# EnricoMiccoli/nodal

Hardware: AMD Instinct MI355X
Metric: circuits_per_sec (higher is better)
Workload: dtype f64; 1 GPU; cfg3: grid(1000) 1e6 nodes, sparse CSR path; n=999999, nnz=4995995, parallelism=one GPU

## Files before the change

nodal_amd/csrc/sagg.hip:

```cpp
#include <hip/hip_ext.h>

#include <atomic>
#include <type_traits>

#include "group.h"

int grounded_flags(nodal_ctx *h, uint8_t *flags_dev);

namespace {

using grp::TB;
constexpr int PW = 4;
constexpr int ACAP = 64;
constexpr int RCAP = 96;
constexpr int RCAP_SMALL = 512;
constexpr int RCAP_SMALL_ROWS = 16384;
inline int rcap_for(int64_t nc) { return nc <= RCAP_SMALL_ROWS ? RCAP_SMALL : RCAP; }
constexpr int W0_MAX = 32;
constexpr int COARSEST = 64;
constexpr int MAX_LEVELS = 12;
constexpr int MIS_ROUNDS = 6;
constexpr int TAIL_MAX_N = 1024;
constexpr int TAIL_LEVELS = 6;
constexpr int TAIL_LDS_BUDGET = 150 * 1024;
// ... 2 lines not shown
#ifndef NODAL_SA_OMEGA
#define NODAL_SA_OMEGA 0.85
#endif
constexpr double OMEGA = NODAL_SA_OMEGA;
constexpr double OMEGA_P = 0.70;
constexpr double OMEGA_P_COARSE = 0.85;
using cyc_t = nodal_cyc_t;

inline unsigned grid_for(int64_t n, unsigned cap = 8192) {
    int64_t g = (n + TB - 1) / TB;
    if (g < 1) g = 1;
    if (g >= 64) g = (g + 7) & ~(int64_t)7;
    return (unsigned)(g > cap ? cap : g);
}
inline int64_t pad64(int64_t n) { return (n + 63) & ~(int64_t)63; }

__device__ __forceinline__ unsigned xcd_block() {
    const unsigned g = gridDim.x, b = blockIdx.x;
    return (g & 7u) ? b : (b & 7u) * (g >> 3) + (b >> 3);
}


struct Ell {
    int64_t n = 0, ld = 0;
    int32_t width = 0;
    const int32_t *col = nullptr;
    const int16_t *dcol = nullptr;
    const double *val = nullptr;
    const float *valf = nullptr;
    const int32_t *len = nullptr;
};

enum { ST_MAXLEN = 0, ST_GRADED = 1, ST_BADDIAG = 2, ST_OVERFLOW = 3, ST_NNZ = 4, ST_UNASSIGNED = 5,
       ST_MAXR = 6, ST_NC = 7 ,
       ST_FARCOL = 8 , ST_COUNT = 9 };

struct SLevel {
    int64_t n = 0, ld = 0, nc = 0;
    int32_t width = 0;
    int32_t maxlen = 0;
    int32_t wfix = 0;
    int64_t nnz = 0;
    DevBuf acol, aval, alen, dinv;
    DevBuf adcol;
    bool d16 = false;
    DevBuf agg, pcol, pval;
    DevBuf rcol, rval, rlen;
    int64_t rld = 0;
    DevBuf vec, part, gflag;
    DevBuf avalf, pvalf, rvalf;
    Ell A() const {
        Ell e;
        e.n = n; e.ld = ld; e.width = width;
        e.col = acol.as<int32_t>(); e.val = aval.as<double>(); e.len = alen.as<int32_t>();
        e.valf = avalf.as<float>();
        e.dcol = d16 ? adcol.as<int16_t>() : nullptr;
        return e;
    }
    template <typename T = double> T *v(int which) const { return reinterpret_cast<T *>(vec.as<double>() + (int64_t)which * ld); }
};
enum { V_X = 0, V_R = 1, V_XP = 2, V_RC = 3, V_C1 = 4, V_C2 = 5, V_V1 = 6, V_V2 = 7, V_R2 = 8, V_X1 = 9, V_T = 10,
       V_COUNT = 11 };

struct TailLevelDesc {
    int n, nc, ld, rld, width, nq, lpr;
// ... 61 lines not shown
        if (it_exec) (void)hipGraphExecDestroy(it_exec);
        if (it_graph) (void)hipGraphDestroy(it_graph);
        it_exec = nullptr;
        it_graph = nullptr;
        it_key = 0;
    }
    ~SHierarchy() {
        drop_graph();
        if (ev_copy) (void)hipEventDestroy(ev_copy);
        if (ev_fork) (void)hipEventDestroy(ev_fork);
        if (ev_join) (void)hipEventDestroy(ev_join);
        if (ev_flags) (void)hipEventDestroy(ev_flags);
        if (aux) (void)hipStreamDestroy(aux);
        for (SLevel *l : pool) {
            DevBuf *b[] = {&l->acol, &l->aval, &l->alen, &l->dinv, &l->agg, &l->pcol, &l->pval, &l->rcol,
                           &l->rval, &l->rlen, &l->vec, &l->part, &l->gflag, &l->avalf, &l->pvalf, &l->rvalf, &l->adcol};
            for (DevBuf *x : b) x->release();
            delete l;
        }
        tail_image.release();
        tail_op.release();
        mvec.release();
        tail_stamps.release();
        bstat.release();
        apcol.release();
        apval.release();
        aplen.release();
        DevBuf *b[] = {&stats, &coarse_inv, &mis_t, &mis_m, &mis_flag, &mis_id, &agg1, &keys, &rstart, &cursor, &lists};
        for (DevBuf *x : b) x->release();
        if (host_stats) (void)hipHostFree(host_stats);
    }
// ... 455 lines not shown
    }
}

__device__ __forceinline__ int wave_excl_scan(int v, int *total) {
    const int lane = threadIdx.x & 63;
    int incl = v;
#pragma unroll
    for (int off = 1; off < 64; off <<= 1) {
        const int t = __shfl_up(incl, off, 64);
        if (lane >= off) incl += t;
    }
    *total = __shfl(incl, 63, 64);
    return incl - v;
}

template <int APW>
__global__ __launch_bounds__(TB) void ap_rows(Ell A, const int32_t *__restrict__ pcol, const double *__restrict__ pval,
                                              int32_t *__restrict__ apcol, double *__restrict__ apval,
                                              int32_t *__restrict__ aplen, unsigned long long *__restrict__ stats) {
    bool overflow = false;
    for (int64_t i = (int64_t)xcd_block() * TB + threadIdx.x; i < A.n; i += (int64_t)gridDim.x * TB) {
        int32_t c[APW];
        double v[APW];
#pragma unroll
        for (int q = 0; q < APW; ++q) { c[q] = -1; v[q] = 0.0; }
        int cnt = 0;
        const int32_t l = A.len[i];
        for (int32_t s = 0; s < l; ++s) {
            const int32_t k = A.col[(int64_t)s * A.ld + i];
            const double a = A.val[(int64_t)s * A.ld + i];
            int32_t J[PW];
            double pp[PW];
#pragma unroll
            for (int sp = 0; sp < PW; ++sp) {
                J[sp] = pcol[(int64_t)sp * A.ld + k];
                pp[sp] = pval[(int64_t)sp * A.ld + k];
            }
#pragma unroll
// ... 5 lines not shown
                for (int q = 0; q < APW; ++q)
                    if (!placed && c[q] == J[sp]) { v[q] += t; placed = true; }
#pragma unroll
                for (int q = 0; q < APW; ++q)
                    if (!placed && c[q] < 0) { c[q] = J[sp]; v[q] = t; placed = true; cnt = q + 1; }
                if (!placed) overflow = true;
            }
        }
#pragma unroll
        for (int q = 0; q < APW; ++q)
            if (q < cnt) {
                apcol[(int64_t)q * A.ld + i] = c[q];
                apval[(int64_t)q * A.ld + i] = v[q];
            }
        aplen[i] = cnt;
    }
    if (overflow) atomicOr(&stats[ST_OVERFLOW], 4ull);
}

template <int APW>
__global__ __launch_bounds__(64) void ap_rows_lds(Ell A, const int32_t *__restrict__ pcol,
                                                  const double *__restrict__ pval, int32_t *__restrict__ apcol,
                                                  double *__restrict__ apval, int32_t *__restrict__ aplen,
                                                  unsigned long long *__restrict__ stats) {
    __shared__ int32_t tc[APW * 64];
    __shared__ double tv[APW * 64];
    const int lane = threadIdx.x;
    bool overflow = false;
    for (int64_t i0 = (int64_t)xcd_block() * 64; i0 < A.n; i0 += (int64_t)gridDim.x * 64) {
        const int64_t i = i0 + lane;
#pragma unroll 8
        for (int q = 0; q < APW; ++q) tc[q * 64 + lane] = -1;
        int cnt = 0;
        if (i < A.n) {
            const int32_t l = A.len[i];
            constexpr int AB = 4;
            for (int32_t s0 = 0; s0 < l; s0 += AB) {
                int32_t kk[AB];
                double aa[AB];
#pragma unroll
                for (int u = 0; u < AB; ++u) {
                    const int32_t su = s0 + u < l ? s0 + u : 0;
                    kk[u] = A.col[(int64_t)su * A.ld + i];
                    aa[u] = A.val[(int64_t)su * A.ld + i];
                }
                int32_t J[AB][PW];
                double pp[AB][PW];
#pragma unroll
                for (int u = 0; u < AB; ++u)
#pragma unroll
// ... 15 lines not shown
                            if (c == J[u][sp]) {
                                tv[slot * 64 + lane] += t;
                                placed = true;
                            } else if (c < 0) {
                                tc[slot * 64 + lane] = J[u][sp];
                                tv[slot * 64 + lane] = t;
                                ++cnt;
                                placed = true;
                            }
                            slot = (slot + 1) & (APW - 1);
                        }
                        if (!placed) overflow = true;
                    }
                }
            }
            int o = 0;
            for (int q = 0; q < APW; ++q) {
                const int32_t c = tc[q * 64 + lane];
                if (c >= 0) {
                    apcol[(int64_t)o * A.ld + i] = c;
                    apval[(int64_t)o * A.ld + i] = tv[q * 64 + lane];
                    ++o;
                }
            }
            aplen[i] = cnt;
        }
    }
    if (overflow) atomicOr(&stats[ST_OVERFLOW], 4ull);
}

__device__ __forceinline__ int galerkin_products(int64_t ld, const int32_t *__restrict__ apcol,
                                                 const double *__restrict__ apval, const int32_t *__restrict__ aplen,
                                                 int64_t rld, const int32_t *__restrict__ rcol,
                                                 const double *__restrict__ rval, int64_t I, int t0, int tn,
                                                 int32_t *lJ, double *lV) {
    const int lane = threadIdx.x;
    int32_t i = 0, len = 0;
    double w = 0.0;
    if (lane < tn) {
        const int t = t0 + lane;
        const int64_t rat = ((int64_t)(t >> 3) * rld + I) * 8 + (t & 7);
        i = rcol[rat];
        w = rval[rat];
// ... 269 lines not shown
    hipStream_t st = h->stream;
    SLevel *L = H->level(l), *C = H->level(l + 1);
    const int64_t n = L->n, ld = L->ld, nc = C->n;
    Ell A = L->A();
    A.width = L->maxlen;
    unsigned long long *dstats = H->stats.as<unsigned long long>();
    const int apw = A.width <= 6 ? 16 : 64;
    NODAL_HIP_TRY(h, H->apcol.reserve((size_t)apw * ld * 4 + 64));
    NODAL_HIP_TRY(h, H->apval.reserve((size_t)apw * ld * 8 + 64));
    NODAL_HIP_TRY(h, H->aplen.reserve((size_t)ld * 4 + 64));
    int32_t *apcol = H->apcol.as<int32_t>(), *aplen = H->aplen.as<int32_t>();
    double *apval = H->apval.as<double>();
    unsigned long long *lst = dstats + (size_t)l * ST_COUNT;
    const unsigned g = grid_for(n);
    if (phase != 2) {
        switch (apw) {
        case 16: ap_rows<16><<<g, TB, 0, st>>>(A, L->pcol.as<int32_t>(), L->pval.as<double>(), apcol, apval, aplen, lst); break;
        default: {
            const unsigned gl = (unsigned)((n + 63) / 64 < 4096 ? (n + 63) / 64 : 4096);
            ap_rows_lds<64><<<gl, 64, 0, st>>>(A, L->pcol.as<int32_t>(), L->pval.as<double>(), apcol, apval, aplen, lst);
        } break;
        }
        NODAL_HIP_TRY(h, hipGetLastError());
    }
    if (phase == 1) return NODAL_OK;
    int G = 1024 / apw;
    G = (G < 8 ? 8 : (G > 64 ? 64 : G));
    static const int g_env = getenv("NODAL_SA_GG") ? atoi(getenv("NODAL_SA_GG")) : 40;
    if (g_env >= 8 && g_env <= 64 && apw == 16) G = g_env & ~7;
    const int pcap = G * apw + 72;
    const size_t lds = 1024 + (size_t)pcap * 12;
    static const int64_t gcap = getenv("NODAL_SA_GCAP") ? atoll(getenv("NODAL_SA_GCAP")) : 16384;
    static const int maxseg = getenv("NODAL_SA_GSEG") ? atoi(getenv("NODAL_SA_GSEG")) : 4;
    const unsigned gg = (unsigned)(nc < gcap ? nc : (gcap < BSTAT_MAX ? gcap : BSTAT_MAX));
    if (r_ready) NODAL_HIP_TRY(h, hipStreamWaitEvent(st, r_ready, 0));
    galerkin<NUMERIC><<<gg, 64, lds, st>>>(
        ld, apcol, apval, aplen, nc, L->rld, L->rcol.as<int32_t>(), L->rval.as<double>(), L->rlen.as<int32_t>(),
// ... 7 lines not shown
}

double omega_p(int level) {
    static double w[2] = {-1.0, -1.0};
    if (w[0] < 0.0) {
        double a = OMEGA_P, b = OMEGA_P_COARSE;
        if (const char *e = getenv("NODAL_SA_OMEGA_P")) {
            a = atof(e);
            const char *c = strchr(e, ',');
            b = c ? atof(c + 1) : a;
        }
        w[1] = b > 0.0 && b < 1.2 ? b : OMEGA_P_COARSE;
        w[0] = a > 0.0 && a < 1.0 ? a : OMEGA_P;
    }
    return w[level > 0 ? 1 : 0];
}

int build_level(nodal_ctx *h, SHierarchy *H, int l, unsigned long long *hs, bool *declined, bool *stop) {
    hipStream_t st = h->stream;
    SLevel *L = H->level(l);
    const int64_t n = L->n, ld = L->ld;
    Ell A = L->A();
    A.width = L->maxlen;
    unsigned long long *dstats = H->stats.as<unsigned long long>();

    NODAL_HIP_TRY(h, H->mis_t.reserve((size_t)n * 8 + 64));
    NODAL_HIP_TRY(h, H->mis_m.reserve((size_t)n * 8 + 64));
    NODAL_HIP_TRY(h, H->mis_flag.reserve((size_t)(n + 1) * 4 + 64));
    NODAL_HIP_TRY(h, H->mis_id.reserve((size_t)(n + 1) * 4 + 64 + scan_tmp_bytes(n + 1)));
    NODAL_HIP_TRY(h, H->agg1.reserve((size_t)n * 4 + 64));
// ... 99 lines not shown
    NODAL_HIP_TRY(h, L->rlen.reserve((size_t)C->ld * 4 + 64));
    NODAL_HIP_TRY(h, C->acol.reserve((size_t)ACAP * C->ld * 4 + 64));
    NODAL_HIP_TRY(h, C->aval.reserve((size_t)ACAP * C->ld * 8 + 64));
    NODAL_HIP_TRY(h, C->avalf.reserve((size_t)ACAP * C->ld * 4 + 64));
    NODAL_HIP_TRY(h, C->alen.reserve((size_t)C->ld * 4 + 64));
    NODAL_HIP_TRY(h, C->dinv.reserve((size_t)C->ld * 8 + 64));
    if (forked && H->want_flags) {
        if (l == 0) NODAL_HIP_TRY(h, L->gflag.reserve((size_t)n + 64));
        NODAL_HIP_TRY(h, C->gflag.reserve((size_t)C->n + 64));
    }
    {
        const int apw = L->maxlen <= 6 ? 16 : 64;
        NODAL_HIP_TRY(h, H->apcol.reserve((size_t)apw * ld * 4 + 64));
        NODAL_HIP_TRY(h, H->apval.reserve((size_t)apw * ld * 8 + 64));
        NODAL_HIP_TRY(h, H->aplen.reserve((size_t)ld * 4 + 64));
    }
    hipStream_t main_st = h->stream;
    struct StreamGuard {
        nodal_ctx *h;
        hipStream_t keep;
        ~StreamGuard() { h->stream = keep; }
    } guard{h, main_st};
    if (forked) {
        NODAL_HIP_TRY(h, hipEventRecord(H->ev_fork, main_st));
        NODAL_HIP_TRY(h, hipStreamWaitEvent(H->aux, H->ev_fork, 0));
        H->aux_pending = true;
        NODAL_TRY(galerkin_product<false>(h, H, l, nullptr, 1));
        h->stream = H->aux;
        st = H->aux;
    }
// ... 125 lines not shown
        NODAL_HIP_TRY(h, hipDeviceGetAttribute(&ncu, hipDeviceAttributeMultiprocessorCount, h->device >= 0 ? h->device : 0));
        if (ncu < 1) ncu = 1;
        cus[dev].store(ncu, std::memory_order_release);
    }
    NODAL_HIP_TRY(h, H->tail_op.reserve((size_t)n * n * 8 + 64));
    const unsigned gr = (unsigned)(n < ncu ? n : ncu);
    double *T = H->tail_op.as<double>();
    const char *img = H->tail_image.as<char>();
    if (d.slots <= 8) k_tail_pack_op<8><<<gr, 1024, (size_t)d.lds_bytes, h->stream>>>(d, img, T);
    else if (d.slots <= 16) k_tail_pack_op<16><<<gr, 1024, (size_t)d.lds_bytes, h->stream>>>(d, img, T);
    else k_tail_pack_op<32><<<gr, 1024, (size_t)d.lds_bytes, h->stream>>>(d, img, T);
    NODAL_HIP_TRY(h, hipGetLastError());
    H->tail_dense = true;
    static const bool check = getenv("NODAL_TRACE") && getenv("NODAL_SA_TAIL_CHECK") && atoi(getenv("NODAL_SA_TAIL_CHECK")) != 0;
    if (check) NODAL_TRY(tail_self_check(h, H));
    return NODAL_OK;
}

int build_tail(nodal_ctx *h, SHierarchy *H, const unsigned long long *hs) {
    H->tail = -1;
    H->tail_dense = false;
    const int last = H->nlev - 1;
    auto up16 = [](int x) { return (x + 15) & ~15; };
    for (int t = 1; t <= last; ++t) {
        if (H->pool[t]->n > TAIL_MAX_N || last - t + 1 > TAIL_LEVELS) continue;
        TailDesc d;
        memset(&d, 0, sizeof d);
        d.nlev = last - t + 1;
        d.nu = getenv("NODAL_SA_TAIL_NU") ? atoi(getenv("NODAL_SA_TAIL_NU")) : 3;
        if (d.nu < 1) d.nu = 1;
// ... 109 lines not shown
        NODAL_TRY(galerkin_product<true>(h, H, l, forked ? H->ev_join : nullptr, forked ? 2 : 0));
        if (forked) H->aux_pending = false;
    }
    const int last = H->nlev - 1;
    if (H->dense_coarsest)
        coarsest_inverse<<<1, 256, 0, st>>>(H->pool[last]->A(), H->coarse_inv.as<double>(), dstats + (size_t)last * ST_COUNT);
    if (H->tail >= 0) k_tail_pack<<<1, 1024, 0, st>>>(H->td, H->tail_image.as<char>());
    NODAL_HIP_TRY(h, hipGetLastError());
    NODAL_TRY(form_tail_op(h, H));
    NODAL_HIP_TRY(h, hipMemcpyAsync(hs, dstats, (size_t)MAX_LEVELS * ST_COUNT * 8, hipMemcpyDeviceToHost, st));
    NODAL_WAIT_STREAM(h, st);
    const int64_t bar = n0 / 100 < 32 ? (n0 / 100 > 0 ? n0 / 100 : 1) : 32;
    if (hs[ST_BADDIAG] || (int64_t)hs[ST_GRADED] >= bar) return NODAL_OK;
    for (int k = 1; k < H->nlev; ++k)
        if (hs[(size_t)k * ST_COUNT + ST_BADDIAG] || hs[(size_t)k * ST_COUNT + ST_OVERFLOW]) return NODAL_OK;
    *ok = true;
    return NODAL_OK;
}

}

void sagg_destroy(nodal_ctx *h) {
    delete static_cast<SHierarchy *>(h->sagg);
    h->sagg = nullptr;
}

static int sagg_setup_csr_body(nodal_ctx *h, int64_t n0, int64_t nnz0, const int32_t *indptr0, const int32_t *indices0,
                               const double *data0, bool general, bool check_floating, bool *accepted, int32_t *floating);

int sagg_setup_csr(nodal_ctx *h, int64_t n0, int64_t nnz0, const int32_t *indptr0, const int32_t *indices0,
// ... 103 lines not shown
                fprintf(stderr, "[sagg] declined at level %d (%lld rows): does not coarsen / over a cap / not positive "
                                "(this level: overflow %llx baddiag %llx; level above: overflow %llx unassigned %llu maxr %llu)\n",
                        l, (long long)L->n, hs[(size_t)l * ST_COUNT + ST_OVERFLOW], hs[(size_t)l * ST_COUNT + ST_BADDIAG],
                        l > 0 ? hs[(size_t)(l - 1) * ST_COUNT + ST_OVERFLOW] : 0ull,
                        l > 0 ? hs[(size_t)(l - 1) * ST_COUNT + ST_UNASSIGNED] : 0ull,
                        l > 0 ? hs[(size_t)(l - 1) * ST_COUNT + ST_MAXR] : 0ull);
            return NODAL_OK;
        }
        if (stop) {
            diag_last = true;
            break;
        }
    }
    H->nlev = l + 1;
    SLevel *last = H->level(l);
    if (H->nlev < 2) return NODAL_OK;
    NODAL_HIP_TRY(h, hipMemcpyAsync(hs, dstats, (size_t)MAX_LEVELS * ST_COUNT * 8, hipMemcpyDeviceToHost, st));
    if (!H->ev_copy) NODAL_HIP_TRY(h, hipEventCreateWithFlags(&H->ev_copy, hipEventDisableTiming));
    NODAL_HIP_TRY(h, hipEventRecord(H->ev_copy, st));
    if (check_floating) {
        if (H->flags_levels == 0) {
            NODAL_HIP_TRY(h, H->level(0)->gflag.reserve((size_t)n0 + 64));
            NODAL_TRY(grounded_flags(h, H->level(0)->gflag.as<uint8_t>()));
        } else {
            NODAL_HIP_TRY(h, hipStreamWaitEvent(st, H->ev_flags, 0));
            H->aux_pending = false;
        }
        for (int k = H->flags_levels; k + 1 < H->nlev; ++k) {
            SLevel *L = H->pool[k], *C = H->pool[k + 1];
            NODAL_HIP_TRY(h, C->gflag.reserve((size_t)C->n + 64));
// ... 45 lines not shown
        NODAL_WAIT_STREAM(h, st);
        if (hs[(size_t)l * ST_COUNT + ST_BADDIAG] & 2ull) {
            if (trace) fprintf(stderr, "[sagg] declined: coarsest matrix not positive definite\n");
            return NODAL_OK;
        }
        *floating = hs[(size_t)(MAX_LEVELS - 1) * ST_COUNT + ST_COUNT - 1] != 0 ? 1 : 0;
    }
    if (trace) {
        fprintf(stderr, "[sagg] levels (rows/entries/longest row/padded width):");
        for (int k = 0; k < H->nlev; ++k)
            fprintf(stderr, " %lld/%lld/%d/%d", (long long)H->pool[k]->n, (long long)H->pool[k]->nnz,
                    H->pool[k]->maxlen, H->pool[k]->wfix);
        fprintf(stderr, "  tail %d (%d register slots)  coarsest %s\n", H->tail, H->tail >= 0 ? H->td.slots : 0,
                H->dense_coarsest ? "dense" : "diagonal");
    }
    H->ready = true;
    *accepted = true;
    H->sym_valid = true;
    H->sym_epoch = h->struct_epoch;
    H->sym_n = n0;
    H->sym_nnz = nnz0;
    H->sym_general = general;
    H->sym_check = check_floating;
    H->sym_floating = *floating;
    memcpy(H->sym_stats, hs, sizeof H->sym_stats);
    return NODAL_OK;
}

int sagg_setup(nodal_ctx *h, bool *accepted, int32_t *floating) {
    return sagg_setup_csr(h, h->n, h->nnz, h->indptr.as<int32_t>(), h->indices.as<int32_t>(), h->data.as<double>(),
// ... 31 lines not shown

template <typename TBV, typename TOUT>
int cycle(nodal_ctx *h, SHierarchy *H, int l, const TBV *b, const cyc_t *x0, TOUT *out, const SolveBufs *sb) {
    hipStream_t st = h->stream;
    SLevel *L = H->pool[l];
    const int64_t n = L->n;
    SLevel *C = H->pool[l + 1];
    const int64_t nc = C->n;
    const Ell A = L->A();
    const double *dinv = L->dinv.as<double>();
    const cyc_t *x = x0;
    cyc_t *r = L->v<cyc_t>(V_R), *xp = L->v<cyc_t>(V_XP);
    const unsigned g = sb ? (unsigned)sb->g0 : grid_for(n);
    const unsigned tb = L->wfix ? TB : TB * LPR_RAGGED;
    const int nu = H->nu[l < 2 ? l : 2];
    if (nu >= 2) {
        cyc_t *x1 = L->v<cyc_t>(V_X1);
        SAGG_DISPATCH_W(L->wfix, (k_post<W, false, TBV, cyc_t><<<g, tb, 0, st>>>(A, dinv, b, x0, x1, nullptr, nullptr, nullptr)));
        x = x1;
    }
    if (nu >= 3) {
        cyc_t *x2 = L->v<cyc_t>(V_T);
        SAGG_DISPATCH_W(L->wfix, (k_post<W, false, TBV, cyc_t><<<g, tb, 0, st>>>(A, dinv, b, x, x2, nullptr, nullptr, nullptr)));
        x = x2;
    }
    SAGG_DISPATCH_W(L->wfix, (k_smooth_residual<W, TBV><<<g, tb, 0, st>>>(A, b, x, r)));
    const bool last = l + 1 == H->tail || l + 1 == H->nlev - 1;
    const double *coef = nullptr;
    if (last) {
        double *rc = C->v<double>(V_RC), *c1 = C->v<double>(V_C1);
        k_restrict<double><<<grid_for(nc * RL), TB, 0, st>>>(nc, L->rld, L->rcol.as<int32_t>(), L->rvalf.as<float>(),
                                                            L->rlen.as<int32_t>(), r, rc, C->dinv.as<double>(), nullptr);
        NODAL_HIP_TRY(h, hipGetLastError());
        NODAL_TRY(last_level(h, H, l + 1, rc, c1));
        k_prolong<double><<<grid_for(n), TB, 0, st>>>(n, L->ld, L->pcol.as<int32_t>(), L->pvalf.as<float>(), x, c1,
                                                     (const double *)nullptr, nullptr, xp);
    } else {
        cyc_t *rc = C->v<cyc_t>(V_RC), *c1 = C->v<cyc_t>(V_C1), *c2 = C->v<cyc_t>(V_C2), *x0c = C->v<cyc_t>(V_X);
        k_restrict<cyc_t><<<grid_for(nc * RL), TB, 0, st>>>(nc, L->rld, L->rcol.as<int32_t>(), L->rvalf.as<float>(),
                                                           L->rlen.as<int32_t>(), r, rc, C->dinv.as<double>(), x0c);
        NODAL_HIP_TRY(h, hipGetLastError());
        int nparts = 0;
        const bool kcycle = l < H->klevels && H->kcycle;
        if (kcycle) {
            cyc_t *v1 = C->v<cyc_t>(V_V1), *v2 = C->v<cyc_t>(V_V2), *r2 = C->v<cyc_t>(V_R2);
            double *part = C->part.as<double>();
            const Ell Ac = C->A();
            const unsigned gd = grid_for(nc, DOT_BLOCKS);
            const unsigned tbc = C->wfix ? TB : TB * LPR_RAGGED;
            nparts = (int)gd;
            double *cf = part + 5 * DOT_BLOCKS;
// ... 12 lines not shown
                NODAL_HIP_TRY(h, hipGetLastError());
                NODAL_TRY((cycle<cyc_t, cyc_t>(h, H, l + 1, r2, x0c, c2, nullptr)));
                SAGG_DISPATCH_W(C->wfix, (k_spmv_dots<W><<<gd, tbc, 0, st>>>(Ac, c2, v2, v1, r2, part + 3 * DOT_BLOCKS,
                                                                            part + 2 * DOT_BLOCKS, part + 4 * DOT_BLOCKS)));
                NODAL_HIP_TRY(h, hipGetLastError());
            }
        } else {
            NODAL_TRY((cycle<cyc_t, cyc_t>(h, H, l + 1, rc, x0c, c1, nullptr)));
        }
        if (nparts) {
            double *cf = C->part.as<double>() + 5 * DOT_BLOCKS;
            const bool sample = l == 0 && H->kslot >= 0;
            k_kcoef<<<1, 320, 0, st>>>(C->part.as<double>(), nparts, cf, sample ? H->kslot : -1, sample ? H->kcount : 0);
            coef = cf;
        }
        k_prolong<cyc_t><<<grid_for(n), TB, 0, st>>>(n, L->ld, L->pcol.as<int32_t>(), L->pvalf.as<float>(), x, c1, c2, coef,
                                                    xp);
    }
    const cyc_t *cur = xp;
    if (nu >= 2) {
        cyc_t *mid = L->v<cyc_t>(V_T);
        SAGG_DISPATCH_W(L->wfix, (k_post<W, false, TBV, cyc_t><<<g, tb, 0, st>>>(A, dinv, b, cur, mid, nullptr, nullptr, nullptr)));
        cur = mid;
    }
    if (nu >= 3) {
        cyc_t *mid2 = L->v<cyc_t>(V_X1);
        SAGG_DISPATCH_W(L->wfix, (k_post<W, false, TBV, cyc_t><<<g, tb, 0, st>>>(A, dinv, b, cur, mid2, nullptr, nullptr, nullptr)));
        cur = mid2;
    }
    if (sb) {
        SAGG_DISPATCH_W(L->wfix, (k_post<W, true, TBV, TOUT><<<g, tb, 0, st>>>(A, dinv, b, cur, out, sb->Ap, sb->part_rz,
                                                                              sb->part_zap)));
    } else {
        SAGG_DISPATCH_W(L->wfix, (k_post<W, false, TBV, TOUT><<<g, tb, 0, st>>>(A, dinv, b, cur, out, nullptr, nullptr, nullptr)));
    }
    NODAL_HIP_TRY(h, hipGetLastError());
    return NODAL_OK;
}

__global__ void f_set_scalars(double *__restrict__ sc, double tol2) {
// ... 170 lines not shown
    };
    static const bool graphs = getenv("NODAL_SA_GRAPH") && atoi(getenv("NODAL_SA_GRAPH")) != 0;
    if (graphs && (H->refreshed || !do_setup)) {
        uint64_t key = 1469598103934665603ull;
        auto mix = [&](uint64_t v) { key = (key ^ v) * 1099511628211ull; };
        mix((uint64_t)(uintptr_t)base); mix((uint64_t)(uintptr_t)x); mix((uint64_t)n); mix((uint64_t)sb.g0);
        mix((uint64_t)H->nlev); mix((uint64_t)(H->tail + 1)); mix((uint64_t)H->kcycle); mix((uint64_t)H->klevels);
        mix((uint64_t)(H->nu[0] * 100 + H->nu[1] * 10 + H->nu[2])); mix((uint64_t)H->td.lds_bytes);
        mix((uint64_t)(uintptr_t)H->tail_image.p); mix((uint64_t)(uintptr_t)H->coarse_inv.p);
        mix((uint64_t)(uintptr_t)(H->tail_dense ? H->tail_op.p : nullptr));
        for (int k = 0; k < H->nlev; ++k) {
            const SLevel *L = H->pool[k];
            const void *ps[] = {L->acol.p, L->aval.p, L->avalf.p, L->alen.p, L->dinv.p, L->pcol.p, L->pvalf.p,
                                L->rcol.p, L->rvalf.p, L->rlen.p, L->vec.p, L->part.p};
            for (const void *q : ps) mix((uint64_t)(uintptr_t)q);
            mix((uint64_t)L->n); mix((uint64_t)L->ld); mix((uint64_t)L->wfix); mix((uint64_t)L->rld);
        }
        if (H->it_exec && H->it_key != key) H->drop_graph();
        if (!H->it_exec) {
            hipGraph_t g = nullptr;
            hipGraphExec_t ex = nullptr;
            if (hipStreamBeginCapture(st, hipStreamCaptureModeThreadLocal) == hipSuccess) {
                int cs = iteration(0, false);
                if (cs == NODAL_OK) cs = iteration(1, false);
                const hipError_t ce = hipStreamEndCapture(st, &g);
                if (cs == NODAL_OK && ce == hipSuccess && g && hipGraphInstantiate(&ex, g, nullptr, nullptr, 0) == hipSuccess) {
                    H->it_graph = g;
                    H->it_exec = ex;
                    H->it_key = key;
                } else {
// ... 106 lines not shown
```

nodal_amd/csrc/sagg_cycle.h:

```cpp
#pragma once

namespace {

constexpr int LPR_RAGGED = 1;
template <int W> struct RowLanes { static constexpr int value = W == 0 ? LPR_RAGGED : 1; };

template <class VT, class XF>
__device__ __forceinline__ double ell_row_lanes(const Ell &A, const VT *__restrict__ val, int64_t i, int sub, XF xf) {
    constexpr int Q = 8;
    const int32_t len = A.len[i];
    double acc = 0.0;
    for (int32_t s0 = sub; s0 < len; s0 += LPR_RAGGED * Q) {
        int32_t c[Q];
        double v[Q];
        if (A.dcol) {
#pragma unroll
            for (int q = 0; q < Q; ++q) {
                const bool ok = s0 + q * LPR_RAGGED < len;
                const int64_t at = (int64_t)(ok ? s0 + q * LPR_RAGGED : s0) * A.ld + i;
                c[q] = (int32_t)i + (int32_t)A.dcol[at];
                const VT loaded = val[at];
                v[q] = ok ? (double)loaded : 0.0;
            }
        } else {
// ... 296 lines not shown
        const TOUT os = (TOUT)fma(OMEGA * dinv[i], bi - s, (double)xp[i]);
        const double o = (double)os;
        out[i] = os;
        if (DOTS) {
            a0 = fma(o, bi, a0);
            a1 = fma(o, u[i], a1);
        }
    }
    if (DOTS) {
        a0 = block_sum<NT>(a0);
        a1 = block_sum<NT>(a1);
        if (threadIdx.x == 0) {
            p_ob[blockIdx.x] = a0;
            p_ou[blockIdx.x] = a1;
        }
    }
}

template <int W>
__global__ __launch_bounds__(TB * RowLanes<W>::value) void k_spmv_dots(Ell A, const cyc_t *__restrict__ c, cyc_t *__restrict__ v,
                                                  const cyc_t *__restrict__ u1, const cyc_t *__restrict__ u2,
                                                  double *__restrict__ p_cv, double *__restrict__ p_cu1,
                                                  double *__restrict__ p_cu2) {
    double a0 = 0.0, a1 = 0.0, a2 = 0.0;
    constexpr int LPR = RowLanes<W>::value, NT = TB * LPR;
    const int sub = threadIdx.x & (LPR - 1);
    for (int64_t t = (int64_t)xcd_block() * NT + threadIdx.x; t / LPR < A.n; t += (int64_t)gridDim.x * NT) {
        const int64_t i = t / LPR;
        const double sd = ell_row_w<W>(A, A.valf, i, sub, [&](int32_t j) { return (double)c[j]; });
        if (sub != 0) continue;
// ... 565 lines not shown
```

Baseline: 158.5 circuits/s.

## Fold first post-smoothing sweep into prolongation via precomputed (I-ωD⁻¹A)P operator

New measurement: 163.0 circuits/s (median of 6 runs). 2.8% higher.

```diff
diff --git a/nodal_amd/csrc/sagg.hip b/nodal_amd/csrc/sagg.hip
--- a/nodal_amd/csrc/sagg.hip
+++ b/nodal_amd/csrc/sagg.hip
@@ -40,6 +40,7 @@
     return (unsigned)(g > cap ? cap : g);
 }
 inline int64_t pad64(int64_t n) { return (n + 63) & ~(int64_t)63; }
+inline size_t align256(size_t x) { return (x + 255) & ~(size_t)255; }
 
 __device__ __forceinline__ unsigned xcd_block() {
     const unsigned g = gridDim.x, b = blockIdx.x;
@@ -59,7 +60,9 @@
 
 enum { ST_MAXLEN = 0, ST_GRADED = 1, ST_BADDIAG = 2, ST_OVERFLOW = 3, ST_NNZ = 4, ST_UNASSIGNED = 5,
        ST_MAXR = 6, ST_NC = 7 ,
-       ST_FARCOL = 8 , ST_COUNT = 9 };
+       ST_FARCOL = 8 ,
+       ST_FOLDMISS = 9 ,
+       ST_COUNT = 10 };
 
 struct SLevel {
     int64_t n = 0, ld = 0, nc = 0;
@@ -75,6 +78,9 @@
     int64_t rld = 0;
     DevBuf vec, part, gflag;
     DevBuf avalf, pvalf, rvalf;
+    DevBuf wcol, wval, wlen;
+    int32_t wslots = 0;
+    bool fold_want = false, fold = false;
     Ell A() const {
         Ell e;
         e.n = n; e.ld = ld; e.width = width;
@@ -166,7 +172,8 @@
         if (aux) (void)hipStreamDestroy(aux);
         for (SLevel *l : pool) {
             DevBuf *b[] = {&l->acol, &l->aval, &l->alen, &l->dinv, &l->agg, &l->pcol, &l->pval, &l->rcol,
-                           &l->rval, &l->rlen, &l->vec, &l->part, &l->gflag, &l->avalf, &l->pvalf, &l->rvalf, &l->adcol};
+                           &l->rval, &l->rlen, &l->vec, &l->part, &l->gflag, &l->avalf, &l->pvalf, &l->rvalf, &l->adcol,
+                           &l->wcol, &l->wval, &l->wlen};
             for (DevBuf *x : b) x->release();
             delete l;
         }
@@ -652,14 +659,26 @@
     return incl - v;
 }
 
-template <int APW>
+template <int APW, bool EMIT>
 __global__ __launch_bounds__(TB) void ap_rows(Ell A, const int32_t *__restrict__ pcol, const double *__restrict__ pval,
                                               int32_t *__restrict__ apcol, double *__restrict__ apval,
-                                              int32_t *__restrict__ aplen, unsigned long long *__restrict__ stats) {
-    bool overflow = false;
+                                              int32_t *__restrict__ aplen, unsigned long long *__restrict__ stats,
+                                              const double *__restrict__ dinv, int32_t *__restrict__ wcol,
+                                              float *__restrict__ wval, int32_t *__restrict__ wlen) {
+    bool overflow = false, miss = false;
     for (int64_t i = (int64_t)xcd_block() * TB + threadIdx.x; i < A.n; i += (int64_t)gridDim.x * TB) {
         int32_t c[APW];
         double v[APW];
+        [[maybe_unused]] int32_t Jo[PW];
+        [[maybe_unused]] double po[PW], wd = 0.0;
+        if constexpr (EMIT) {
+#pragma unroll
+            for (int sp = 0; sp < PW; ++sp) {
+                Jo[sp] = pcol[(int64_t)sp * A.ld + i];
+                po[sp] = pval[(int64_t)sp * A.ld + i];
+            }
+            wd = OMEGA * dinv[i];
+        }
 #pragma unroll
         for (int q = 0; q < APW; ++q) { c[q] = -1; v[q] = 0.0; }
         int cnt = 0;
@@ -695,19 +714,39 @@
                 apval[(int64_t)q * A.ld + i] = v[q];
             }
         aplen[i] = cnt;
+        if constexpr (EMIT) {
+            int have = 0, found = 0;
+#pragma unroll
+            for (int sp = 0; sp < PW; ++sp) have += Jo[sp] >= 0 ? 1 : 0;
+#pragma unroll
+            for (int q = 0; q < APW; ++q)
+                if (q < cnt) {
+                    double pv = 0.0;
+#pragma unroll
+                    for (int sp = 0; sp < PW; ++sp)
+                        if (Jo[sp] == c[q]) { pv += po[sp]; ++found; }
+                    wcol[(int64_t)q * A.ld + i] = c[q];
+                    wval[(int64_t)q * A.ld + i] = (float)(pv - wd * v[q]);
+                }
+            wlen[i] = cnt;
+            if (found != have) miss = true;
+        }
     }
     if (overflow) atomicOr(&stats[ST_OVERFLOW], 4ull);
-}
-
-template <int APW>
+    if (miss) stats[ST_FOLDMISS] = 1ull;
+}
+
+template <int APW, bool EMIT>
 __global__ __launch_bounds__(64) void ap_rows_lds(Ell A, const int32_t *__restrict__ pcol,
                                                   const double *__restrict__ pval, int32_t *__restrict__ apcol,
                                                   double *__restrict__ apval, int32_t *__restrict__ aplen,
-                                                  unsigned long long *__restrict__ stats) {
+                                                  unsigned long long *__restrict__ stats,
+                                                  const double *__restrict__ dinv, int32_t *__restrict__ wcol,
+                                                  float *__restrict__ wval, int32_t *__restrict__ wlen) {
     __shared__ int32_t tc[APW * 64];
     __shared__ double tv[APW * 64];
     const int lane = threadIdx.x;
-    bool overflow = false;
+    bool overflow = false, miss = false;
     for (int64_t i0 = (int64_t)xcd_block() * 64; i0 < A.n; i0 += (int64_t)gridDim.x * 64) {
         const int64_t i = i0 + lane;
 #pragma unroll 8
@@ -715,6 +754,16 @@
         int cnt = 0;
         if (i < A.n) {
             const int32_t l = A.len[i];
+            [[maybe_unused]] int32_t Jo[PW];
+            [[maybe_unused]] double po[PW], wd = 0.0;
+            if constexpr (EMIT) {
+#pragma unroll
+                for (int sp = 0; sp < PW; ++sp) {
+                    Jo[sp] = pcol[(int64_t)sp * A.ld + i];
+                    po[sp] = pval[(int64_t)sp * A.ld + i];
+                }
+                wd = OMEGA * dinv[i];
+            }
             constexpr int AB = 4;
             for (int32_t s0 = 0; s0 < l; s0 += AB) {
                 int32_t kk[AB];
@@ -760,19 +809,36 @@
                     }
                 }
             }
-            int o = 0;
+            int o = 0, found = 0;
             for (int q = 0; q < APW; ++q) {
                 const int32_t c = tc[q * 64 + lane];
                 if (c >= 0) {
+                    const double t = tv[q * 64 + lane];
                     apcol[(int64_t)o * A.ld + i] = c;
-                    apval[(int64_t)o * A.ld + i] = tv[q * 64 + lane];
+                    apval[(int64_t)o * A.ld + i] = t;
+                    if constexpr (EMIT) {
+                        double pv = 0.0;
+#pragma unroll
+                        for (int sp = 0; sp < PW; ++sp)
+                            if (Jo[sp] == c) { pv += po[sp]; ++found; }
+                        wcol[(int64_t)o * A.ld + i] = c;
+                        wval[(int64_t)o * A.ld + i] = (float)(pv - wd * t);
+                    }
                     ++o;
                 }
             }
             aplen[i] = cnt;
+            if constexpr (EMIT) {
+                int have = 0;
+#pragma unroll
+                for (int sp = 0; sp < PW; ++sp) have += Jo[sp] >= 0 ? 1 : 0;
+                wlen[i] = cnt;
+                if (found != have) miss = true;
+            }
         }
     }
     if (overflow) atomicOr(&stats[ST_OVERFLOW], 4ull);
+    if (miss) stats[ST_FOLDMISS] = 1ull;
 }
 
 __device__ __forceinline__ int galerkin_products(int64_t ld, const int32_t *__restrict__ apcol,
@@ -1072,13 +1138,17 @@
     unsigned long long *lst = dstats + (size_t)l * ST_COUNT;
     const unsigned g = grid_for(n);
     if (phase != 2) {
-        switch (apw) {
-        case 16: ap_rows<16><<<g, TB, 0, st>>>(A, L->pcol.as<int32_t>(), L->pval.as<double>(), apcol, apval, aplen, lst); break;
-        default: {
-            const unsigned gl = (unsigned)((n + 63) / 64 < 4096 ? (n + 63) / 64 : 4096);
-            ap_rows_lds<64><<<gl, 64, 0, st>>>(A, L->pcol.as<int32_t>(), L->pval.as<double>(), apcol, apval, aplen, lst);
-        } break;
-        }
+        const bool w = L->fold_want && L->wslots == apw;
+        int32_t *wcol = w ? L->wcol.as<int32_t>() : nullptr, *wlen = w ? L->wlen.as<int32_t>() : nullptr;
+        float *wval = w ? L->wval.as<float>() : nullptr;
+        const double *dinv = L->dinv.as<double>();
+        const int32_t *pc = L->pcol.as<int32_t>();
+        const double *pv = L->pval.as<double>();
+        const unsigned gl = (unsigned)((n + 63) / 64 < 4096 ? (n + 63) / 64 : 4096);
+        if (apw == 16 && w) ap_rows<16, true><<<g, TB, 0, st>>>(A, pc, pv, apcol, apval, aplen, lst, dinv, wcol, wval, wlen);
+        else if (apw == 16) ap_rows<16, false><<<g, TB, 0, st>>>(A, pc, pv, apcol, apval, aplen, lst, dinv, wcol, wval, wlen);
+        else if (w) ap_rows_lds<64, true><<<gl, 64, 0, st>>>(A, pc, pv, apcol, apval, aplen, lst, dinv, wcol, wval, wlen);
+        else ap_rows_lds<64, false><<<gl, 64, 0, st>>>(A, pc, pv, apcol, apval, aplen, lst, dinv, wcol, wval, wlen);
         NODAL_HIP_TRY(h, hipGetLastError());
     }
     if (phase == 1) return NODAL_OK;
@@ -1116,6 +1186,49 @@
         w[0] = a > 0.0 && a < 1.0 ? a : OMEGA_P;
     }
     return w[level > 0 ? 1 : 0];
+}
+
+constexpr int64_t FOLD_MAX_ROWS = 1 << 19;
+struct FoldSetting { int mode = 0; unsigned mask = 0; };
+const FoldSetting &fold_setting() {
+    static const FoldSetting s = [] {
+        FoldSetting f;
+        const char *e = getenv("NODAL_SA_FOLD_POST");
+        if (!e || !*e) return f;
+        if (strchr(e, 'l')) {
+            f.mode = 3;
+            for (const char *q = e; (q = strchr(q, 'l')) != nullptr; ++q) {
+                const int k = atoi(q + 1);
+                if (q[1] >= '0' && q[1] <= '9' && k < MAX_LEVELS) f.mask |= 1u << k;
+            }
+        } else {
+            f.mode = atoi(e) == 0 ? 1 : 2;
+        }
+        return f;
+    }();
+    return s;
+}
+bool fold_wanted(int level, int64_t n) {
+    if (level > 0 && n <= TAIL_MAX_N) return false;
+    const FoldSetting &f = fold_setting();
+    switch (f.mode) {
+    case 1: return false;
+    case 2: return true;
+    case 3: return (f.mask >> level & 1u) != 0;
+    default: return n <= FOLD_MAX_ROWS;
+    }
+}
+void decide_folds(SHierarchy *H, const unsigned long long *hs, bool trace) {
+    for (int k = 0; k < H->nlev; ++k) {
+        SLevel *L = H->pool[k];
+        const bool runs_cycle = k + 1 < H->nlev && (H->tail < 0 || k < H->tail);
+        const bool miss = hs[(size_t)k * ST_COUNT + ST_FOLDMISS] != 0;
+        L->fold = L->fold_want && runs_cycle && !miss;
+        if (trace && L->fold_want && runs_cycle)
+            fprintf(stderr, "[sagg] level %d (%lld rows): first post-smoothing sweep %s\n", k, (long long)L->n,
+                    miss ? "NOT folded: a row of A P lacks a column of its P row (no stored diagonal)"
+                         : "folded into the prolongation");
+    }
 }
 
 int build_level(nodal_ctx *h, SHierarchy *H, int l, unsigned long long *hs, bool *declined, bool *stop) {
@@ -1245,6 +1358,14 @@
         NODAL_HIP_TRY(h, H->apcol.reserve((size_t)apw * ld * 4 + 64));
         NODAL_HIP_TRY(h, H->apval.reserve((size_t)apw * ld * 8 + 64));
         NODAL_HIP_TRY(h, H->aplen.reserve((size_t)ld * 4 + 64));
+        L->fold = false;
+        L->fold_want = fold_wanted(l, n);
+        L->wslots = apw;
+        if (L->fold_want) {
+            NODAL_HIP_TRY(h, L->wcol.reserve((size_t)apw * ld * 4 + 64));
+            NODAL_HIP_TRY(h, L->wval.reserve((size_t)apw * ld * 4 + 64));
+            NODAL_HIP_TRY(h, L->wlen.reserve((size_t)ld * 4 + 64));
+        }
     }
     hipStream_t main_st = h->stream;
     struct StreamGuard {
@@ -1400,6 +1521,80 @@
     H->tail_dense = true;
     static const bool check = getenv("NODAL_TRACE") && getenv("NODAL_SA_TAIL_CHECK") && atoi(getenv("NODAL_SA_TAIL_CHECK")) != 0;
     if (check) NODAL_TRY(tail_self_check(h, H));
+    return NODAL_OK;
+}
+
+template <typename TC>
+int fold_check_level(nodal_ctx *h, SHierarchy *H, int l, bool two) {
+    hipStream_t st = h->stream;
+    const SLevel *L = H->pool[l];
+    const int64_t n = L->n, nc = H->pool[l + 1]->n;
+    const Ell A = L->A();
+    uint64_t seed = 0x9e3779b97f4a7c15ull + (uint64_t)l;
+    auto unit = [&]() {
+        uint64_t z = (seed += 0x9e3779b97f4a7c15ull);
+        z = (z ^ (z >> 30)) * 0xbf58476d1ce4e5b9ull;
+        z = (z ^ (z >> 27)) * 0x94d049bb133111ebull;
+        z ^= z >> 31;
+        return (double)(z >> 11) * (1.0 / 4503599627370496.0) - 1.0;
+    };
+    std::vector<cyc_t> hx((size_t)n), hb((size_t)n);
+    std::vector<TC> he((size_t)2 * nc);
+    for (auto &v : hx) v = (cyc_t)unit();
+    for (auto &v : hb) v = (cyc_t)unit();
+    for (auto &v : he) v = (TC)unit();
+    const double hcoef[2] = {0.9, 0.4};
+    const size_t vb = align256((size_t)n * sizeof(cyc_t)), eb = align256((size_t)nc * sizeof(TC)), db = align256((size_t)n * 8);
+    DevBuf buf;
+    hipError_t e = buf.reserve(6 * vb + 2 * eb + 2 * db + 256);
+    char *p = buf.as<char>();
+    cyc_t *x = reinterpret_cast<cyc_t *>(p), *b = reinterpret_cast<cyc_t *>(p + vb), *r = reinterpret_cast<cyc_t *>(p + 2 * vb),
+          *xp = reinterpret_cast<cyc_t *>(p + 3 * vb), *mt = reinterpret_cast<cyc_t *>(p + 4 * vb),
+          *mf = reinterpret_cast<cyc_t *>(p + 5 * vb);
+    TC *c1 = reinterpret_cast<TC *>(p + 6 * vb), *c2 = reinterpret_cast<TC *>(p + 6 * vb + eb);
+    double *d = reinterpret_cast<double *>(p + 6 * vb + 2 * eb), *q = reinterpret_cast<double *>(p + 6 * vb + 2 * eb + db);
+    double *coef = reinterpret_cast<double *>(p + 6 * vb + 2 * eb + 2 * db);
+    std::vector<double> hd((size_t)n), hq((size_t)n);
+    if (e == hipSuccess) e = hipMemcpyAsync(x, hx.data(), (size_t)n * sizeof(cyc_t), hipMemcpyHostToDevice, st);
+    if (e == hipSuccess) e = hipMemcpyAsync(b, hb.data(), (size_t)n * sizeof(cyc_t), hipMemcpyHostToDevice, st);
+    if (e == hipSuccess) e = hipMemcpyAsync(c1, he.data(), (size_t)nc * sizeof(TC), hipMemcpyHostToDevice, st);
+    if (e == hipSuccess) e = hipMemcpyAsync(c2, he.data() + nc, (size_t)nc * sizeof(TC), hipMemcpyHostToDevice, st);
+    if (e == hipSuccess) e = hipMemcpyAsync(coef, hcoef, sizeof hcoef, hipMemcpyHostToDevice, st);
+    if (e == hipSuccess) {
+        const unsigned g = grid_for(n), tb = L->wfix ? TB : TB * LPR_RAGGED;
+        const double *dinv = L->dinv.as<double>(), *cf = two ? coef : nullptr;
+        const int32_t *wcol = L->wcol.as<int32_t>(), *wlen = L->wlen.as<int32_t>();
+        const float *wval = L->wval.as<float>();
+        SAGG_DISPATCH_W(L->wfix, (k_smooth_residual<W, cyc_t><<<g, tb, 0, st>>>(A, b, x, r)));
+        k_prolong<TC><<<g, TB, 0, st>>>(n, L->ld, L->pcol.as<int32_t>(), L->pvalf.as<float>(), x, c1, two ? c2 : nullptr, cf, xp);
+        SAGG_DISPATCH_W(L->wfix, (k_post<W, false, cyc_t, cyc_t><<<g, tb, 0, st>>>(A, dinv, b, xp, mt, nullptr, nullptr, nullptr)));
+        k_prolong_post<TC, cyc_t><<<g, TB, 0, st>>>(n, L->ld, wcol, wval, wlen, x, r, dinv, c1, two ? c2 : nullptr, cf, mf);
+        k_fold_check<TC><<<g, TB, 0, st>>>(A, dinv, b, x, xp, wcol, wval, wlen, c1, two ? c2 : nullptr, cf, mt, mf, d, q);
+        e = hipGetLastError();
+    }
+    if (e == hipSuccess) e = hipStreamSynchronize(st);
+    if (e == hipSuccess) e = hipMemcpy(hd.data(), d, (size_t)n * 8, hipMemcpyDeviceToHost);
+    if (e == hipSuccess) e = hipMemcpy(hq.data(), q, (size_t)n * 8, hipMemcpyDeviceToHost);
+    buf.release();
+    NODAL_HIP_TRY(h, e);
+    double dm = 0.0, qm = 0.0;
+    for (int64_t i = 0; i < n; ++i) {
+        dm = !(hd[i] <= dm) ? hd[i] : dm;
+        qm = !(hq[i] <= qm) ? hq[i] : qm;
+    }
+    fprintf(stderr, "[sagg] fold check: level %d, rows %lld, slots %d, width %d, fused launch against the two d = %.3e "
+                    "(worst row against its own bound: %.3e)\n", l, (long long)n, (int)L->wslots, (int)L->maxlen, dm, qm);
+    return NODAL_OK;
+}
+int fold_self_check(nodal_ctx *h, SHierarchy *H) {
+    static const bool check = getenv("NODAL_TRACE") && getenv("NODAL_SA_FOLD_CHECK") && atoi(getenv("NODAL_SA_FOLD_CHECK")) != 0;
+    if (!check) return NODAL_OK;
+    for (int l = 0; l + 1 < H->nlev; ++l) {
+        if (!H->pool[l]->fold) continue;
+        const bool last = l + 1 == H->tail || l + 1 == H->nlev - 1;
+        if (last) NODAL_TRY(fold_check_level<double>(h, H, l, false));
+        else NODAL_TRY(fold_check_level<cyc_t>(h, H, l, true));
+    }
     return NODAL_OK;
 }
 
@@ -1539,6 +1734,8 @@
     if (hs[ST_BADDIAG] || (int64_t)hs[ST_GRADED] >= bar) return NODAL_OK;
     for (int k = 1; k < H->nlev; ++k)
         if (hs[(size_t)k * ST_COUNT + ST_BADDIAG] || hs[(size_t)k * ST_COUNT + ST_OVERFLOW]) return NODAL_OK;
+    decide_folds(H, hs, false);
+    NODAL_TRY(fold_self_check(h, H));
     *ok = true;
     return NODAL_OK;
 }
@@ -1672,6 +1869,7 @@
     }
     H->nlev = l + 1;
     SLevel *last = H->level(l);
+    last->fold_want = last->fold = false;
     if (H->nlev < 2) return NODAL_OK;
     NODAL_HIP_TRY(h, hipMemcpyAsync(hs, dstats, (size_t)MAX_LEVELS * ST_COUNT * 8, hipMemcpyDeviceToHost, st));
     if (!H->ev_copy) NODAL_HIP_TRY(h, hipEventCreateWithFlags(&H->ev_copy, hipEventDisableTiming));
@@ -1747,6 +1945,8 @@
         fprintf(stderr, "  tail %d (%d register slots)  coarsest %s\n", H->tail, H->tail >= 0 ? H->td.slots : 0,
                 H->dense_coarsest ? "dense" : "diagonal");
     }
+    decide_folds(H, hs, trace);
+    NODAL_TRY(fold_self_check(h, H));
     H->ready = true;
     *accepted = true;
     H->sym_valid = true;
@@ -1808,6 +2008,18 @@
     const unsigned g = sb ? (unsigned)sb->g0 : grid_for(n);
     const unsigned tb = L->wfix ? TB : TB * LPR_RAGGED;
     const int nu = H->nu[l < 2 ? l : 2];
+    const bool fold = L->fold && !(sb && nu == 1);
+    auto hand_up = [&](const auto *c1, const auto *c2, const double *cf) {
+        using TC = std::remove_cv_t<std::remove_pointer_t<decltype(c1)>>;
+        if (!fold)
+            k_prolong<TC><<<grid_for(n), TB, 0, st>>>(n, L->ld, L->pcol.as<int32_t>(), L->pvalf.as<float>(), x, c1, c2, cf, xp);
+        else if (nu == 1)
+            k_prolong_post<TC, TOUT><<<grid_for(n), TB, 0, st>>>(n, L->ld, L->wcol.as<int32_t>(), L->wval.as<float>(),
+                                                               L->wlen.as<int32_t>(), x, r, dinv, c1, c2, cf, out);
+        else
+            k_prolong_post<TC, cyc_t><<<grid_for(n), TB, 0, st>>>(n, L->ld, L->wcol.as<int32_t>(), L->wval.as<float>(),
+                                                                L->wlen.as<int32_t>(), x, r, dinv, c1, c2, cf, xp);
+    };
     if (nu >= 2) {
         cyc_t *x1 = L->v<cyc_t>(V_X1);
         SAGG_DISPATCH_W(L->wfix, (k_post<W, false, TBV, cyc_t><<<g, tb, 0, st>>>(A, dinv, b, x0, x1, nullptr, nullptr, nullptr)));
@@ -1827,8 +2039,7 @@
                                                             L->rlen.as<int32_t>(), r, rc, C->dinv.as<double>(), nullptr);
         NODAL_HIP_TRY(h, hipGetLastError());
         NODAL_TRY(last_level(h, H, l + 1, rc, c1));
-        k_prolong<double><<<grid_for(n), TB, 0, st>>>(n, L->ld, L->pcol.as<int32_t>(), L->pvalf.as<float>(), x, c1,
-                                                     (const double *)nullptr, nullptr, xp);
+        hand_up((const double *)c1, (const double *)nullptr, nullptr);
     } else {
         cyc_t *rc = C->v<cyc_t>(V_RC), *c1 = C->v<cyc_t>(V_C1), *c2 = C->v<cyc_t>(V_C2), *x0c = C->v<cyc_t>(V_X);
         k_restrict<cyc_t><<<grid_for(nc * RL), TB, 0, st>>>(nc, L->rld, L->rcol.as<int32_t>(), L->rvalf.as<float>(),
@@ -1871,16 +2082,20 @@
             k_kcoef<<<1, 320, 0, st>>>(C->part.as<double>(), nparts, cf, sample ? H->kslot : -1, sample ? H->kcount : 0);
             coef = cf;
         }
-        k_prolong<cyc_t><<<grid_for(n), TB, 0, st>>>(n, L->ld, L->pcol.as<int32_t>(), L->pvalf.as<float>(), x, c1, c2, coef,
-                                                    xp);
+        hand_up((const cyc_t *)c1, (const cyc_t *)c2, coef);
     }
     const cyc_t *cur = xp;
-    if (nu >= 2) {
+    const int left = fold ? nu - 1 : nu;
+    if (left == 0) {
+        NODAL_HIP_TRY(h, hipGetLastError());
+        return NODAL_OK;
+    }
+    if (left >= 2) {
         cyc_t *mid = L->v<cyc_t>(V_T);
         SAGG_DISPATCH_W(L->wfix, (k_post<W, false, TBV, cyc_t><<<g, tb, 0, st>>>(A, dinv, b, cur, mid, nullptr, nullptr, nullptr)));
         cur = mid;
     }
-    if (nu >= 3) {
+    if (left >= 3) {
         cyc_t *mid2 = L->v<cyc_t>(V_X1);
         SAGG_DISPATCH_W(L->wfix, (k_post<W, false, TBV, cyc_t><<<g, tb, 0, st>>>(A, dinv, b, cur, mid2, nullptr, nullptr, nullptr)));
         cur = mid2;
@@ -2081,6 +2296,8 @@
             const void *ps[] = {L->acol.p, L->aval.p, L->avalf.p, L->alen.p, L->dinv.p, L->pcol.p, L->pvalf.p,
                                 L->rcol.p, L->rvalf.p, L->rlen.p, L->vec.p, L->part.p};
             for (const void *q : ps) mix((uint64_t)(uintptr_t)q);
+            mix((uint64_t)(L->fold ? 1 + L->wslots : 0));
+            if (L->fold) { mix((uint64_t)(uintptr_t)L->wcol.p); mix((uint64_t)(uintptr_t)L->wval.p); mix((uint64_t)(uintptr_t)L->wlen.p); }
             mix((uint64_t)L->n); mix((uint64_t)L->ld); mix((uint64_t)L->wfix); mix((uint64_t)L->rld);
         }
         if (H->it_exec && H->it_key != key) H->drop_graph();
diff --git a/nodal_amd/csrc/sagg_cycle.h b/nodal_amd/csrc/sagg_cycle.h
--- a/nodal_amd/csrc/sagg_cycle.h
+++ b/nodal_amd/csrc/sagg_cycle.h
@@ -334,6 +334,70 @@
             p_ob[blockIdx.x] = a0;
             p_ou[blockIdx.x] = a1;
         }
+    }
+}
+
+template <typename TC, typename TOUT>
+__global__ __launch_bounds__(TB) void k_prolong_post(int64_t n, int64_t ld, const int32_t *__restrict__ wcol,
+                                                     const float *__restrict__ wval, const int32_t *__restrict__ wlen,
+                                                     const cyc_t *__restrict__ x, const cyc_t *__restrict__ r,
+                                                     const double *__restrict__ dinv, const TC *__restrict__ c1,
+                                                     const TC *__restrict__ c2, const double *__restrict__ coef,
+                                                     TOUT *__restrict__ out) {
+    constexpr int Q = 8;
+    const bool two = coef != nullptr;
+    const double s1 = two ? coef[0] : 1.0, s2 = two ? coef[1] : 0.0;
+    for (int64_t i = (int64_t)xcd_block() * TB + threadIdx.x; i < n; i += (int64_t)gridDim.x * TB) {
+        const int32_t len = wlen[i];
+        const cyc_t xi = x[i], ri = r[i];
+        const double di = dinv[i];
+        double acc = 0.0;
+        for (int32_t s0 = 0; s0 < len; s0 += Q) {
+            int32_t J[Q];
+            double w[Q];
+#pragma unroll
+            for (int q = 0; q < Q; ++q) {
+                const bool ok = s0 + q < len;
+                const int64_t at = (int64_t)(ok ? s0 + q : s0) * ld + i;
+                J[q] = wcol[at];
+                const float loaded = wval[at];
+                w[q] = ok ? (double)loaded : 0.0;
+            }
+#pragma unroll
+            for (int q = 0; q < Q; ++q) {
+                const double e = two ? s1 * (double)c1[J[q]] + s2 * (double)c2[J[q]] : (double)c1[J[q]];
+                acc = fma(w[q], e, acc);
+            }
+        }
+        out[i] = (TOUT)(fma(OMEGA * di, (double)ri, (double)xi) + acc);
+    }
+}
+
+template <typename TC>
+__global__ __launch_bounds__(TB) void k_fold_check(Ell A, const double *__restrict__ dinv, const cyc_t *__restrict__ b,
+                                                   const cyc_t *__restrict__ x, const cyc_t *__restrict__ xp,
+                                                   const int32_t *__restrict__ wcol, const float *__restrict__ wval,
+                                                   const int32_t *__restrict__ wlen, const TC *__restrict__ c1,
+                                                   const TC *__restrict__ c2, const double *__restrict__ coef,
+                                                   const cyc_t *__restrict__ m_two, const cyc_t *__restrict__ m_fused,
+                                                   double *__restrict__ d, double *__restrict__ q) {
+    const bool two = coef != nullptr;
+    const double s1 = two ? coef[0] : 1.0, s2 = two ? coef[1] : 0.0;
+    for (int64_t i = (int64_t)xcd_block() * TB + threadIdx.x; i < A.n; i += (int64_t)gridDim.x * TB) {
+        double ax = 0.0, we = 0.0;
+        const int32_t la = A.len[i], lw = wlen[i];
+        for (int32_t s = 0; s < la; ++s)
+            ax += fabs((double)A.valf[(int64_t)s * A.ld + i]) * fabs((double)xp[A.col[(int64_t)s * A.ld + i]]);
+        for (int32_t s = 0; s < lw; ++s) {
+            const int32_t j = wcol[(int64_t)s * A.ld + i];
+            const double e = two ? s1 * (double)c1[j] + s2 * (double)c2[j] : (double)c1[j];
+            we += fabs((double)wval[(int64_t)s * A.ld + i]) * fabs(e);
+        }
+        const double den = fabs((double)x[i]) + OMEGA * dinv[i] * (fabs((double)b[i]) + ax) + we;
+        const double diff = fabs((double)m_fused[i] - (double)m_two[i]);
+        const double di = diff / den;
+        d[i] = di;
+        q[i] = di / ((double)(lw + la + 8) * 0x1p-23);
     }
 }
 
```
